# jhbastek/PhysicsInformedDiffusionModels

Measured on NVIDIA H100. Metric: train samples/s Darcy 64x64 PIDM, higher is better.
Workload: dtype bf16

## Files before the change

physicsinformeddiffusionmodels_b200/csrc/attention_fused.cu:

```cuda
#define PIDM_PDL_GROUP 1
#include "common.cuh"
#include "mma_util.cuh"
#include "pidm.h"

namespace pidm {

constexpr int LF_C = 32;

__device__ __forceinline__ uint32_t movm_t(uint32_t x) {
    uint32_t y;
    asm volatile("movmatrix.sync.aligned.m8n8.trans.b16 %0, %1;" : "=r"(y) : "r"(x));
    return y;
}

__device__ __forceinline__ void load_w_frags(uint32_t (&w)[2][4][2], const __nv_bfloat16* __restrict__ Wrows, int lane) {
    const int g = lane >> 2, t = lane & 3;
#pragma unroll
    for (int ks = 0; ks < 2; ++ks)
#pragma unroll
        for (int nt = 0; nt < 4; ++nt) {
            const uint32_t* row = reinterpret_cast<const uint32_t*>(Wrows + (size_t)(nt * 8 + g) * LF_C + ks * 16 + 2 * t);
            w[ks][nt][0] = __ldg(row);
            w[ks][nt][1] = __ldg(row + 4);
        }
}
template <int MT>
__device__ __forceinline__ void load_x_frags(uint32_t (&a)[MT][2][4], const __nv_bfloat16* Xs, int lane) {
#pragma unroll
    for (int mt = 0; mt < MT; ++mt)
#pragma unroll
        for (int ks = 0; ks < 2; ++ks) frag_a_rowmajor(a[mt][ks], Xs, LW_PITCH, mt * 16, ks * 16, lane);
}
template <int MT>
__device__ __forceinline__ void project(float (&c)[MT][4][4], const uint32_t (&a)[MT][2][4], const uint32_t (&w)[2][4][2]) {
#pragma unroll
    for (int mt = 0; mt < MT; ++mt)
#pragma unroll
        for (int nt = 0; nt < 4; ++nt) {
#pragma unroll
            for (int i = 0; i < 4; ++i) c[mt][nt][i] = 0.f;
#pragma unroll
            for (int ks = 0; ks < 2; ++ks) mma_bf16(c[mt][nt], a[mt][ks], w[ks][nt][0], w[ks][nt][1]);
        }
}
__device__ __forceinline__ void frag_softmax(float (&c)[4][4], float mul) {
#pragma unroll
    for (int half = 0; half < 2; ++half) {
        float mx = -INFINITY;
#pragma unroll
        for (int nt = 0; nt < 4; ++nt) mx = fmaxf(mx, fmaxf(c[nt][half * 2], c[nt][half * 2 + 1]));
        mx = fmaxf(mx, __shfl_xor_sync(0xffffffffu, mx, 1));
        mx = fmaxf(mx, __shfl_xor_sync(0xffffffffu, mx, 2));
        float s = 0.f;
#pragma unroll
        for (int nt = 0; nt < 4; ++nt) {
            c[nt][half * 2] = __expf(c[nt][half * 2] - mx);
            c[nt][half * 2 + 1] = __expf(c[nt][half * 2 + 1] - mx);
            s += c[nt][half * 2] + c[nt][half * 2 + 1];
        }
        s += __shfl_xor_sync(0xffffffffu, s, 1);
        s += __shfl_xor_sync(0xffffffffu, s, 2);
        const float inv = mul / s;
#pragma unroll
        for (int nt = 0; nt < 4; ++nt) { c[nt][half * 2] *= inv; c[nt][half * 2 + 1] *= inv; }
    }
}
__device__ __forceinline__ void c_to_a(uint32_t (&a)[2][4], const float (&c)[4][4]) {
#pragma unroll
    for (int ks = 0; ks < 2; ++ks) {
        a[ks][0] = pack_bf16(c[2 * ks][0], c[2 * ks][1]);
        a[ks][1] = pack_bf16(c[2 * ks][2], c[2 * ks][3]);
        a[ks][2] = pack_bf16(c[2 * ks + 1][0], c[2 * ks + 1][1]);
        a[ks][3] = pack_bf16(c[2 * ks + 1][2], c[2 * ks + 1][3]);
    }
}
__device__ __forceinline__ void load_cols(float (&v)[8], const float* __restrict__ src, int lane) {
    const int t = lane & 3;
#pragma unroll
    for (int nt = 0; nt < 4; ++nt) { v[nt * 2] = src[nt * 8 + 2 * t]; v[nt * 2 + 1] = src[nt * 8 + 2 * t + 1]; }
}

constexpr int LFS_STAGES = 2;
__global__ void __launch_bounds__(256) laf_kmax_kernel(const __nv_bfloat16* __restrict__ xn,
                                                       const __nv_bfloat16* __restrict__ W, float* __restrict__ part,
                                                       int N, int rows_per_chunk) {
    pdl_trigger();
    pdl_wait();
    extern __shared__ __align__(16) unsigned char raw[];
    const int b = blockIdx.y, chunk = blockIdx.x, lane = threadIdx.x & 31, h = threadIdx.x >> 5;
    __nv_bfloat16* ring = reinterpret_cast<__nv_bfloat16*>(raw) + (size_t)h * (LFS_STAGES * LW_TILE);
    const int n_begin = chunk * rows_per_chunk, n_end = min(N, n_begin + rows_per_chunk);
    const int n_tiles = (n_end - n_begin) / 32;
    const __nv_bfloat16* xsrc = xn + ((size_t)b * N + n_begin) * LF_C;
    auto issue = [&](int it) {
        if (it < n_tiles) lw_issue<32>(ring + (size_t)(it % LFS_STAGES) * LW_TILE, xsrc + (size_t)it * 32 * LF_C, LF_C, lane);
        cp_commit();
    };
#pragma unroll
    for (int s = 0; s < LFS_STAGES; ++s) issue(s);
    uint32_t wk[2][4][2];
    load_w_frags(wk, W + (size_t)(LM_HID + h * LM_D) * LF_C, lane);
    float m[8];
#pragma unroll
    for (int i = 0; i < 8; ++i) m[i] = -INFINITY;
    for (int it = 0; it < n_tiles; ++it) {
        cp_wait<LFS_STAGES - 1>();
        __syncwarp();
        uint32_t ax[2][2][4];
        load_x_frags<2>(ax, ring + (size_t)(it % LFS_STAGES) * LW_TILE, lane);
        __syncwarp();
        issue(it + LFS_STAGES);
        float ck[2][4][4];
        project<2>(ck, ax, wk);
#pragma unroll
        for (int nt = 0; nt < 4; ++nt)
#pragma unroll
            for (int j = 0; j < 2; ++j)
                m[nt * 2 + j] = fmaxf(fmaxf(m[nt * 2 + j], fmaxf(ck[0][nt][j], ck[0][nt][2 + j])),
                                      fmaxf(ck[1][nt][j], ck[1][nt][2 + j]));
    }
#pragma unroll
    for (int off = 4; off < 32; off <<= 1)
#pragma unroll
        for (int i = 0; i < 8; ++i) m[i] = fmaxf(m[i], __shfl_xor_sync(0xffffffffu, m[i], off));
    if (lane < 4) {
        float* o = part + ((size_t)b * gridDim.x + chunk) * LM_HID + h * LM_D;
#pragma unroll
        for (int nt = 0; nt < 4; ++nt)
#pragma unroll
            for (int j = 0; j < 2; ++j) o[nt * 8 + 2 * lane + j] = m[nt * 2 + j];
    }
}

__global__ void laf_finalize_kernel(float* __restrict__ ctx, float* __restrict__ kzinv, int n_rows) {
    pdl_trigger();
    pdl_wait();
    const int row = blockIdx.x * (blockDim.x / 32) + (threadIdx.x >> 5), lane = threadIdx.x & 31;
    if (row >= n_rows) return;
    const float zi = 1.f / kzinv[row];
    ctx[(size_t)row * LM_D + lane] *= zi;
    __syncwarp();
    if (lane == 0) kzinv[row] = zi;
}

constexpr int LFP_WO_TILE = LF_C * LW_PITCH;

__device__ __forceinline__ void lfp_dout_acc(float (&c)[4][4], const uint32_t (&ady)[2][4], const __nv_bfloat16* Wo, int lane) {
#pragma unroll
    for (int nt = 0; nt < 4; ++nt)
#pragma unroll
        for (int i = 0; i < 4; ++i) c[nt][i] = 0.f;
#pragma unroll
    for (int kc = 0; kc < 2; ++kc)
#pragma unroll
        for (int np = 0; np < 2; ++np) {
            uint32_t bw[4];
            frag_b_krows(bw, Wo, LW_PITCH, kc * 16, np * 16, lane);
            mma_bf16(c[2 * np], ady[kc], bw[0], bw[1]);
            mma_bf16(c[2 * np + 1], ady[kc], bw[2], bw[3]);
        }
}
__device__ __forceinline__ void lfp_dout(uint32_t (&ag)[2][4], const __nv_bfloat16* dyt, const __nv_bfloat16* Wo, int lane) {
    uint32_t ady[2][4];
    frag_a_rowmajor(ady[0], dyt, LW_PITCH, 0, 0, lane);
    frag_a_rowmajor(ady[1], dyt, LW_PITCH, 0, 16, lane);
    float c[4][4];
    lfp_dout_acc(c, ady, Wo, lane);
    c_to_a(ag, c);
}

template <int MODE, bool PROJ = false>
struct LfcCfg {
    static constexpr int STAGES = MODE == 0 ? 4 : 2;
    static constexpr int STAGE_ELEMS = MODE == 0 ? LW_TILE : 2 * LW_TILE;
    static constexpr size_t SMEM = (size_t)LM_HEADS * STAGES * STAGE_ELEMS * 2 + (size_t)LM_HEADS * 2 * LM_D * 4 +
                                   (PROJ ? (size_t)LM_HEADS * LFP_WO_TILE * 2 : 0);
};
template <int MODE, bool PROJ = false>
__global__ void __launch_bounds__(256, 2) laf_ctx_kernel(const __nv_bfloat16* __restrict__ xn, const __nv_bfloat16* __restrict__ W,
                                                      const __nv_bfloat16* __restrict__ dout, const float* __restrict__ part,
                                                      int n_stat_chunks, float* __restrict__ kmax, float* __restrict__ kzinv,
                                                      float* __restrict__ ctx, int N, int chunk_px, float scale,
                                                      const __nv_bfloat16* __restrict__ w_out) {
    static_assert(!PROJ || MODE == 1, "PROJ applies to the dcontext pass");
    pdl_trigger();
    pdl_wait();
    extern __shared__ __align__(16) unsigned char raw[];
    constexpr int LFC_STAGES = LfcCfg<MODE>::STAGES, LFC_STAGE_ELEMS = LfcCfg<MODE>::STAGE_ELEMS;
    const int b = blockIdx.y, chunk = blockIdx.x, lane = threadIdx.x & 31, h = threadIdx.x >> 5;
    __nv_bfloat16* ring = reinterpret_cast<__nv_bfloat16*>(raw) + (size_t)h * (LFC_STAGES * LFC_STAGE_ELEMS);
    float* sM = reinterpret_cast<float*>(raw + (size_t)LM_HEADS * LFC_STAGES * LFC_STAGE_ELEMS * 2) + h * 2 * LM_D;
    float* sZi = sM + LM_D;
    __nv_bfloat16* Wo = reinterpret_cast<__nv_bfloat16*>(raw + LfcCfg<MODE>::SMEM) + h * LFP_WO_TILE;
    const int n_begin = chunk * chunk_px, n_end = min(N, n_begin + chunk_px);
    const int n_tiles = (n_end - n_begin) / 32;
    const size_t pix0 = (size_t)b * N + n_begin;
    const __nv_bfloat16* xsrc = xn + pix0 * LF_C;
    const __nv_bfloat16* gsrc = (MODE == 1) ? (PROJ ? dout + pix0 * LF_C : dout + pix0 * LM_HID + h * LM_D) : nullptr;
    constexpr int G_STRIDE = PROJ ? LF_C : LM_HID;
    if (PROJ) {
        lw_issue<32>(Wo, w_out + h * LM_D, LM_HID, lane);
        cp_commit();
    }
    auto issue = [&](int it) {
        if (it < n_tiles) {
            __nv_bfloat16* buf = ring + (size_t)(it % LFC_STAGES) * LFC_STAGE_ELEMS;
            lw_issue<32>(buf, xsrc + (size_t)it * 32 * LF_C, LF_C, lane);
            if (MODE == 1) lw_issue<32>(buf + LW_TILE, gsrc + (size_t)it * 32 * G_STRIDE, G_STRIDE, lane);
        }
        cp_commit();
    };
#pragma unroll
    for (int s = 0; s < LFC_STAGES; ++s) issue(s);
    uint32_t w0[2][4][2], w1[2][4][2];
    load_w_frags(w0, W + (size_t)((MODE == 0 ? LM_HID : 0) + h * LM_D) * LF_C, lane);
    if (MODE == 0) load_w_frags(w1, W + (size_t)(2 * LM_HID + h * LM_D) * LF_C, lane);
    float Mc[8];
    float zacc[8];
#pragma unroll
    for (int i = 0; i < 8; ++i) zacc[i] = 0.f;
    if (MODE == 0) {
        const int c = h * LM_D + lane;
        float M = -INFINITY;
        for (int i = 0; i < n_stat_chunks; ++i) M = fmaxf(M, part[((size_t)b * n_stat_chunks + i) * LM_HID + c]);
        sM[lane] = M;
        if (chunk == 0) kmax[(size_t)b * LM_HID + c] = M;
        __syncwarp();
        load_cols(Mc, sM, lane);
    }
    float acc[2][4][4];
#pragma unroll
    for (int i = 0; i < 2; ++i)
#pragma unroll
        for (int j = 0; j < 4; ++j)
#pragma unroll
            for (int k = 0; k < 4; ++k) acc[i][j][k] = 0.f;
    for (int it = 0; it < n_tiles; ++it) {
        cp_wait<LFC_STAGES - 1>();
        __syncwarp();
        const __nv_bfloat16* buf = ring + (size_t)(it % LFC_STAGES) * LFC_STAGE_ELEMS;
        uint32_t ax[2][2][4];
        load_x_frags<2>(ax, buf, lane);
        uint32_t bv[2][4][2];
        if (PROJ) {
#pragma unroll
            for (int mt = 0; mt < 2; ++mt) {
                uint32_t ady[2][4];
                frag_a_rowmajor(ady[0], buf + LW_TILE, LW_PITCH, mt * 16, 0, lane);
                frag_a_rowmajor(ady[1], buf + LW_TILE, LW_PITCH, mt * 16, 16, lane);
                float cd[4][4];
                lfp_dout_acc(cd, ady, Wo, lane);
#pragma unroll
                for (int nt = 0; nt < 4; ++nt) {
                    bv[mt][nt][0] = movm_t(pack_bf16(cd[nt][0], cd[nt][1]));
                    bv[mt][nt][1] = movm_t(pack_bf16(cd[nt][2], cd[nt][3]));
                }
            }
        } else if (MODE == 1) {
#pragma unroll
            for (int ks = 0; ks < 2; ++ks) {
                uint32_t b01[4], b23[4];
                frag_b_krows(b01, buf + LW_TILE, LW_PITCH, ks * 16, 0, lane);
                frag_b_krows(b23, buf + LW_TILE, LW_PITCH, ks * 16, 16, lane);
                bv[ks][0][0] = b01[0]; bv[ks][0][1] = b01[1]; bv[ks][1][0] = b01[2]; bv[ks][1][1] = b01[3];
                bv[ks][2][0] = b23[0]; bv[ks][2][1] = b23[1]; bv[ks][3][0] = b23[2]; bv[ks][3][1] = b23[3];
            }
        }
        __syncwarp();
        issue(it + LFC_STAGES);
        float cw[2][4][4];
        project<2>(cw, ax, w0);
        if (MODE == 0) {
#pragma unroll
            for (int mt = 0; mt < 2; ++mt)
#pragma unroll
                for (int nt = 0; nt < 4; ++nt)
#pragma unroll
                    for (int i = 0; i < 4; ++i) {
                        cw[mt][nt][i] = __expf(cw[mt][nt][i] - Mc[nt * 2 + (i & 1)]);
                        zacc[nt * 2 + (i & 1)] += cw[mt][nt][i];
                    }
            float cv[2][4][4];
            project<2>(cv, ax, w1);
#pragma unroll
            for (int mt = 0; mt < 2; ++mt)
#pragma unroll
                for (int nt = 0; nt < 4; ++nt) {
                    bv[mt][nt][0] = movm_t(pack_bf16(cv[mt][nt][0], cv[mt][nt][1]));
                    bv[mt][nt][1] = movm_t(pack_bf16(cv[mt][nt][2], cv[mt][nt][3]));
                }
        } else {
            frag_softmax(cw[0], scale);
            frag_softmax(cw[1], scale);
        }
#pragma unroll
        for (int mt = 0; mt < 2; ++mt) {
#pragma unroll
            for (int md = 0; md < 2; ++md) {
                uint32_t a[4];
                a[0] = movm_t(pack_bf16(cw[mt][2 * md][0], cw[mt][2 * md][1]));
                a[1] = movm_t(pack_bf16(cw[mt][2 * md + 1][0], cw[mt][2 * md + 1][1]));
                a[2] = movm_t(pack_bf16(cw[mt][2 * md][2], cw[mt][2 * md][3]));
                a[3] = movm_t(pack_bf16(cw[mt][2 * md + 1][2], cw[mt][2 * md + 1][3]));
#pragma unroll
                for (int ne = 0; ne < 4; ++ne) mma_bf16(acc[md][ne], a, bv[mt][ne][0], bv[mt][ne][1]);
            }
        }
    }
    const int g = lane >> 2, t = lane & 3;
    if (MODE == 0) {
#pragma unroll
        for (int off = 4; off < 32; off <<= 1)
#pragma unroll
            for (int i = 0; i < 8; ++i) zacc[i] += __shfl_xor_sync(0xffffffffu, zacc[i], off);
        if (lane < 4) {
#pragma unroll
            for (int nt = 0; nt < 4; ++nt)
#pragma unroll
                for (int j = 0; j < 2; ++j)
                    atomicAdd(kzinv + (size_t)b * LM_HID + h * LM_D + nt * 8 + 2 * lane + j, zacc[nt * 2 + j]);
        }
    }
    float* cb = ctx + ((size_t)b * LM_HEADS + h) * LM_D * LM_D;
#pragma unroll
    for (int md = 0; md < 2; ++md)
#pragma unroll
        for (int half = 0; half < 2; ++half) {
            const int d = md * 16 + g + half * 8;
            const float f = (MODE == 0) ? 1.f / (float)N : 1.f;
#pragma unroll
            for (int ne = 0; ne < 4; ++ne) {
                const int e = ne * 8 + 2 * t;
                atomicAdd(cb + d * LM_D + e, acc[md][ne][half * 2] * f);
                atomicAdd(cb + d * LM_D + e + 1, acc[md][ne][half * 2 + 1] * f);
            }
        }
}

constexpr int LFO_STAGES = 2;
constexpr int LFOP_STAGES = 3;
constexpr int LFO_R_PITCH = LF_C + 8;
constexpr size_t LAF_OUT_PROJ_SMEM = (size_t)LFOP_STAGES * LW_TILE * 2 + (size_t)LM_HEADS * LFP_WO_TILE * 2 +
                                     (size_t)LM_HEADS * 32 * LFO_R_PITCH * 4;
template <bool PROJ = false>
__global__ void __launch_bounds__(256) laf_out_kernel(const __nv_bfloat16* __restrict__ xn, const __nv_bfloat16* __restrict__ W,
                                                      const float* __restrict__ ctx, __nv_bfloat16* __restrict__ out, int N,
                                                      int chunk_px, float scale, const __nv_bfloat16* __restrict__ w_out,
                                                      const float* __restrict__ b_out,
                                                      const __nv_bfloat16* __restrict__ residual) {
    pdl_trigger();
    pdl_wait();
    extern __shared__ __align__(16) unsigned char raw[];
    constexpr int STAGES = PROJ ? LFOP_STAGES : LFO_STAGES;
    const int b = blockIdx.y, chunk = blockIdx.x, lane = threadIdx.x & 31, h = threadIdx.x >> 5;
    __nv_bfloat16* ring = reinterpret_cast<__nv_bfloat16*>(raw) + (PROJ ? 0 : (size_t)h * ((LFO_STAGES + 1) * LW_TILE));
    __nv_bfloat16* Os = ring + LFO_STAGES * LW_TILE;
    __nv_bfloat16* Wo = reinterpret_cast<__nv_bfloat16*>(raw) + LFOP_STAGES * LW_TILE + h * LFP_WO_TILE;
    float* R = reinterpret_cast<float*>(reinterpret_cast<__nv_bfloat16*>(raw) + LFOP_STAGES * LW_TILE +
                                        LM_HEADS * LFP_WO_TILE);
    const int n_begin = chunk * chunk_px, n_end = min(N, n_begin + chunk_px);
    const int n_tiles = (n_end - n_begin) / 32;
    const size_t pix0 = (size_t)b * N + n_begin;
    const __nv_bfloat16* xsrc = xn + pix0 * LF_C;
    __nv_bfloat16* odst = out + pix0 * LM_HID + h * LM_D;
    if (PROJ) {
        lw_issue<32>(Wo, w_out + h * LM_D, LM_HID, lane);
        cp_commit();
    }
    auto issue = [&](int it) {
        if (it < n_tiles && (!PROJ || h == 0))
            lw_issue<32>(ring + (size_t)(it % STAGES) * LW_TILE, xsrc + (size_t)it * 32 * LF_C, LF_C, lane);
        cp_commit();
    };
#pragma unroll
    for (int s = 0; s < (PROJ ? STAGES - 1 : STAGES); ++s) issue(s);
    uint32_t wq[2][4][2];
    load_w_frags(wq, W + (size_t)(h * LM_D) * LF_C, lane);
    const float* ch = ctx + ((size_t)b * LM_HEADS + h) * LM_D * LM_D;
    uint32_t bf[2][4][2];
#pragma unroll
    for (int ks = 0; ks < 2; ++ks)
#pragma unroll
        for (int nt = 0; nt < 4; ++nt) frag_b_global<true>(bf[ks][nt], ch, ks * 16, nt * 8, lane);
    const int g = lane >> 2, t = lane & 3;
    const int rrow = threadIdx.x >> 4, rcol = (threadIdx.x & 15) * 2;
    float2 bias = make_float2(0.f, 0.f);
    if (PROJ) bias = make_float2(b_out[rcol], b_out[rcol + 1]);
    float* Rw = R + h * 32 * LFO_R_PITCH;
    for (int it = 0; it < n_tiles; ++it) {
        uint32_t ax[2][2][4];
        if (PROJ) {
            cp_wait<STAGES - 2>();
            __syncthreads();
            issue(it + STAGES - 1);
            load_x_frags<2>(ax, ring + (size_t)(it % STAGES) * LW_TILE, lane);
        } else {
            cp_wait<LFO_STAGES - 1>();
            __syncwarp();
            load_x_frags<2>(ax, ring + (size_t)(it % LFO_STAGES) * LW_TILE, lane);
            __syncwarp();
            issue(it + LFO_STAGES);
        }
        __nv_bfloat162 res[2];
        if (PROJ)
#pragma unroll
            for (int rh = 0; rh < 2; ++rh)
                res[rh] = *reinterpret_cast<const __nv_bfloat162*>(residual + (pix0 + (size_t)it * 32 + rrow + rh * 16) * LF_C + rcol);
        float cq[2][4][4];
        project<2>(cq, ax, wq);
#pragma unroll
        for (int mt = 0; mt < 2; ++mt) {
            frag_softmax(cq[mt], scale);
            uint32_t a[2][4];
            c_to_a(a, cq[mt]);
            float c[4][4];
#pragma unroll
            for (int i = 0; i < 4; ++i)
#pragma unroll
                for (int k = 0; k < 4; ++k) c[i][k] = 0.f;
#pragma unroll
            for (int ks = 0; ks < 2; ++ks)
#pragma unroll
                for (int nt = 0; nt < 4; ++nt) mma_bf16(c[nt], a[ks], bf[ks][nt][0], bf[ks][nt][1]);
            if (PROJ) {
                c_to_a(a, c);
                float y[4][4];
#pragma unroll
                for (int i = 0; i < 4; ++i)
#pragma unroll
                    for (int k = 0; k < 4; ++k) y[i][k] = 0.f;
#pragma unroll
                for (int ke = 0; ke < 2; ++ke)
#pragma unroll
                    for (int np = 0; np < 2; ++np) {
                        uint32_t bw[4];
                        frag_b_nrows(bw, Wo, LW_PITCH, np * 16, ke * 16, lane);
                        mma_bf16(y[2 * np], a[ke], bw[0], bw[1]);
                        mma_bf16(y[2 * np + 1], a[ke], bw[2], bw[3]);
                    }
#pragma unroll
                for (int nt = 0; nt < 4; ++nt)
#pragma unroll
                    for (int half = 0; half < 2; ++half)
                        *reinterpret_cast<float2*>(Rw + (mt * 16 + g + half * 8) * LFO_R_PITCH + nt * 8 + 2 * t) =
                            make_float2(y[nt][half * 2], y[nt][half * 2 + 1]);
            } else {
#pragma unroll
                for (int nt = 0; nt < 4; ++nt) {
                    __nv_bfloat16* o = Os + (size_t)(mt * 16 + g) * LW_PITCH + nt * 8 + 2 * t;
                    *reinterpret_cast<uint32_t*>(o) = pack_bf16(c[nt][0], c[nt][1]);
                    *reinterpret_cast<uint32_t*>(o + 8 * LW_PITCH) = pack_bf16(c[nt][2], c[nt][3]);
                }
            }
        }
        if (PROJ) {
            __syncthreads();
#pragma unroll
            for (int rh = 0; rh < 2; ++rh) {
                const int row = rrow + rh * 16;
                const size_t pix = pix0 + (size_t)it * 32 + row;
                const float2 x = __bfloat1622float2(res[rh]);
                float sx = x.x + bias.x, sy = x.y + bias.y;
#pragma unroll
                for (int w = 0; w < LM_HEADS; ++w) {
                    const float2 v = *reinterpret_cast<const float2*>(R + (w * 32 + row) * LFO_R_PITCH + rcol);
                    sx += v.x;
                    sy += v.y;
                }
                *reinterpret_cast<uint32_t*>(out + pix * LF_C + rcol) = pack_bf16(sx, sy);
            }
        } else {
            __syncwarp();
            lw_store<32>(odst + (size_t)it * 32 * LM_HID, LM_HID, Os, lane);
            __syncwarp();
        }
    }
}

constexpr int LFB_ROWS = 16;
constexpr int LFB_STAGES = 4;
constexpr int LFB_TILE = LFB_ROWS * LW_PITCH;

struct LfbTile {
    uint32_t ax[1][2][4], ag[2][4];
};
__device__ __forceinline__ void lfb_dq(float (&dq)[4][4], const LfbTile& tl, const uint32_t (&wq)[2][4][2],
                                       const uint32_t (&bc)[2][4][2], float scale) {
    float c1[1][4][4], c2[4][4];
    project<1>(c1, tl.ax, wq);
    frag_softmax(c1[0], 1.f);
#pragma unroll
    for (int nt = 0; nt < 4; ++nt) {
#pragma unroll
        for (int i = 0; i < 4; ++i) c2[nt][i] = 0.f;
#pragma unroll
        for (int ks = 0; ks < 2; ++ks) mma_bf16(c2[nt], tl.ag[ks], bc[ks][nt][0], bc[ks][nt][1]);
    }
#pragma unroll
    for (int half = 0; half < 2; ++half) {
        float dot = 0.f;
#pragma unroll
        for (int nt = 0; nt < 4; ++nt)
            dot += c1[0][nt][half * 2] * c2[nt][half * 2] + c1[0][nt][half * 2 + 1] * c2[nt][half * 2 + 1];
        dot += __shfl_xor_sync(0xffffffffu, dot, 1);
        dot += __shfl_xor_sync(0xffffffffu, dot, 2);
#pragma unroll
        for (int nt = 0; nt < 4; ++nt)
#pragma unroll
            for (int j = 0; j < 2; ++j) dq[nt][half * 2 + j] = scale * c1[0][nt][half * 2 + j] * (c2[nt][half * 2 + j] - dot);
    }
}
__device__ __forceinline__ void lfb_dkdv(float (&dk)[4][4], float (&dv)[4][4], const uint32_t (&ax)[1][2][4],
                                         const uint32_t (&wk)[2][4][2], const uint32_t (&wv)[2][4][2],
                                         const uint32_t (&bd)[2][4][2], const uint32_t (&bt)[2][4][2],
                                         const float (&Mc)[8], const float (&Zc)[8], const float (&cdc)[8], float invN) {
    float c1[1][4][4];
    uint32_t a[2][4];
    project<1>(c1, ax, wv);
    c_to_a(a, c1[0]);
#pragma unroll
    for (int nt = 0; nt < 4; ++nt) {
#pragma unroll
        for (int i = 0; i < 4; ++i) dk[nt][i] = 0.f;
#pragma unroll
        for (int ks = 0; ks < 2; ++ks) mma_bf16(dk[nt], a[ks], bd[ks][nt][0], bd[ks][nt][1]);
    }
    project<1>(c1, ax, wk);
#pragma unroll
    for (int nt = 0; nt < 4; ++nt)
#pragma unroll
        for (int i = 0; i < 4; ++i) {
            c1[0][nt][i] = __expf(c1[0][nt][i] - Mc[nt * 2 + (i & 1)]) * Zc[nt * 2 + (i & 1)];
            dk[nt][i] = c1[0][nt][i] * (dk[nt][i] * invN - cdc[nt * 2 + (i & 1)]);
        }
    c_to_a(a, c1[0]);
#pragma unroll
    for (int nt = 0; nt < 4; ++nt) {
#pragma unroll
        for (int i = 0; i < 4; ++i) dv[nt][i] = 0.f;
#pragma unroll
        for (int ks = 0; ks < 2; ++ks) mma_bf16(dv[nt], a[ks], bt[ks][nt][0], bt[ks][nt][1]);
#pragma unroll
        for (int i = 0; i < 4; ++i) dv[nt][i] *= invN;
    }
}
__device__ __forceinline__ void lfb_cd(float (&cdc)[8], float* scd, const float* __restrict__ cg, const float* __restrict__ dg,
                                       int lane) {
    float s = 0.f;
#pragma unroll
    for (int e = 0; e < LM_D; e += 4) {
        const float4 x = *reinterpret_cast<const float4*>(dg + lane * LM_D + e);
        const float4 y = *reinterpret_cast<const float4*>(cg + lane * LM_D + e);
        s += x.x * y.x + x.y * y.y + x.z * y.z + x.w * y.w;
    }
    scd[lane] = s;
    __syncwarp();
    load_cols(cdc, scd, lane);
}

constexpr int LFB_W_PITCH = LF_C + 8;
constexpr int LFB_R_PITCH = LF_C + 8;
template <bool PROJ>
struct LfbCfg {
    static constexpr int STAGE_ELEMS = (PROJ ? 2 : 1 + LM_HEADS) * LFB_TILE;
    static constexpr size_t SMEM_BASE = (size_t)LFB_STAGES * STAGE_ELEMS * 2 + (size_t)3 * LM_HID * LFB_W_PITCH * 2 +
                                        (size_t)LM_HEADS * LFB_ROWS * LFB_R_PITCH * 4 + (size_t)LM_HEADS * LM_D * 4;
    static constexpr size_t SMEM = SMEM_BASE + (PROJ ? (size_t)LM_HEADS * LFP_WO_TILE * 2 : 0);
};

__device__ __forceinline__ void mma_w(float (&c)[4][4], const uint32_t (&g)[2][4], const __nv_bfloat16* Wh, int lane) {
#pragma unroll
    for (int kd = 0; kd < 2; ++kd)
#pragma unroll
        for (int np = 0; np < 2; ++np) {
            uint32_t bw[4];
            frag_b_krows(bw, Wh, LFB_W_PITCH, kd * 16, np * 16, lane);
            mma_bf16(c[2 * np], g[kd], bw[0], bw[1]);
            mma_bf16(c[2 * np + 1], g[kd], bw[2], bw[3]);
        }
}

template <bool PROJ = false>
__global__ void __launch_bounds__(256) laf_bwd_kernel(const __nv_bfloat16* __restrict__ xn, const __nv_bfloat16* __restrict__ W,
                                                      const __nv_bfloat16* __restrict__ dout, const float* __restrict__ ctx,
                                                      const float* __restrict__ dctx, const float* __restrict__ kmax,
                                                      const float* __restrict__ kzinv, __nv_bfloat16* __restrict__ dxn,
                                                      int N, int chunk_px, float scale, const __nv_bfloat16* __restrict__ w_out) {
    pdl_trigger();
    pdl_wait();
    extern __shared__ __align__(16) unsigned char raw[];
    constexpr int LFB_STAGE_ELEMS = LfbCfg<PROJ>::STAGE_ELEMS;
    const int b = blockIdx.y, chunk = blockIdx.x, lane = threadIdx.x & 31, h = threadIdx.x >> 5;
    __nv_bfloat16* ring = reinterpret_cast<__nv_bfloat16*>(raw);
    __nv_bfloat16* Ws = ring + LFB_STAGES * LFB_STAGE_ELEMS;
    __nv_bfloat16* Wo = reinterpret_cast<__nv_bfloat16*>(raw + LfbCfg<PROJ>::SMEM_BASE) + h * LFP_WO_TILE;
    float* R = reinterpret_cast<float*>(Ws + 3 * LM_HID * LFB_W_PITCH);
    float* scd = R + LM_HEADS * LFB_ROWS * LFB_R_PITCH + h * LM_D;
    const int n_begin = chunk * chunk_px, n_end = min(N, n_begin + chunk_px);
// ... 116 lines not shown
        for (int np = 0; np < 2; ++np) {
            mma_bf16(acc[md][2 * np], a, bx[np][0], bx[np][1]);
            mma_bf16(acc[md][2 * np + 1], a, bx[np][2], bx[np][3]);
        }
    }
}

template <int PART, bool PROJ = false>
__global__ void __launch_bounds__(256) laf_wgrad_kernel(const __nv_bfloat16* __restrict__ xn, const __nv_bfloat16* __restrict__ W,
                                                        const __nv_bfloat16* __restrict__ dout, const float* __restrict__ ctx,
                                                        const float* __restrict__ dctx, const float* __restrict__ kmax,
                                                        const float* __restrict__ kzinv, float* __restrict__ grad_w, int N,
                                                        int chunk_px, long long w_stride_n, long long w_stride_c, float scale,
                                                        const __nv_bfloat16* __restrict__ w_out, float* __restrict__ grad_wo,
                                                        long long wo_stride_n, long long wo_stride_c) {
    pdl_trigger();
    pdl_wait();
    extern __shared__ __align__(16) unsigned char raw[];
    using Cfg = LfwCfg<PART, PROJ>;
    constexpr int MATS = Cfg::MATS, STAGE_ELEMS = Cfg::STAGE_ELEMS, S_PITCH = Cfg::S_PITCH;
    const int b = blockIdx.y, chunk = blockIdx.x, lane = threadIdx.x & 31, h = threadIdx.x >> 5;
    __nv_bfloat16* ring = reinterpret_cast<__nv_bfloat16*>(raw) + (size_t)h * (LFB_STAGES * STAGE_ELEMS);
    float* scd = reinterpret_cast<float*>(raw + (size_t)LM_HEADS * LFB_STAGES * STAGE_ELEMS * 2) + h * LM_D;
    __nv_bfloat16* Wo = reinterpret_cast<__nv_bfloat16*>(raw + Cfg::SMEM_BASE) + h * LFP_WO_TILE;
    const int n_begin = chunk * chunk_px, n_end = min(N, n_begin + chunk_px);
    const int n_tiles = (n_end - n_begin) / LFB_ROWS;
    const size_t pix0 = (size_t)b * N + n_begin;
    const __nv_bfloat16* xsrc = xn + pix0 * LF_C;
    const __nv_bfloat16* gsrc = PROJ ? dout + pix0 * LF_C : dout + pix0 * LM_HID + h * LM_D;
    constexpr int G_STRIDE = PROJ ? LF_C : LM_HID;
    if (PROJ) {
        lw_issue<32>(Wo, w_out + h * LM_D, LM_HID, lane);
        cp_commit();
    }
    auto issue = [&](int it) {
        if (it < n_tiles) {
            __nv_bfloat16* buf = ring + (size_t)(it % LFB_STAGES) * STAGE_ELEMS;
            lw_issue<LFB_ROWS>(buf, xsrc + (size_t)it * LFB_ROWS * LF_C, LF_C, lane);
            if (PART == 0) lw_issue<LFB_ROWS>(buf + LFB_TILE, gsrc + (size_t)it * LFB_ROWS * G_STRIDE, G_STRIDE, lane);
        }
        cp_commit();
    };
#pragma unroll
    for (int s = 0; s < LFB_STAGES; ++s) issue(s);
    const float* cg = ctx + ((size_t)b * LM_HEADS + h) * LM_D * LM_D;
    const float* dg = dctx + ((size_t)b * LM_HEADS + h) * LM_D * LM_D;
    float Mc[8], Zc[8], cdc[8];
    uint32_t w0[2][4][2], w1[2][4][2];
    uint32_t b0[2][4][2], b1[2][4][2];
    if (PART == 0) {
        load_w_frags(w0, W + (size_t)(h * LM_D) * LF_C, lane);
    } else {
        lfb_cd(cdc, scd, cg, dg, lane);
        load_cols(Mc, kmax + (size_t)b * LM_HID + h * LM_D, lane);
        load_cols(Zc, kzinv + (size_t)b * LM_HID + h * LM_D, lane);
        load_w_frags(w0, W + (size_t)(LM_HID + h * LM_D) * LF_C, lane);
        load_w_frags(w1, W + (size_t)(2 * LM_HID + h * LM_D) * LF_C, lane);
    }
#pragma unroll
    for (int ks = 0; ks < 2; ++ks)
#pragma unroll
        for (int nt = 0; nt < 4; ++nt) {
            frag_b_global<false>(b0[ks][nt], PART == 0 ? cg : dg, ks * 16, nt * 8, lane);
            if (PART == 1 || PROJ) frag_b_global<true>(b1[ks][nt], PART == 1 ? dg : cg, ks * 16, nt * 8, lane);
        }
    const float invN = 1.f / (float)N;
    float acc[MATS][2][4][4];
#pragma unroll
    for (int m = 0; m < MATS; ++m)
#pragma unroll
        for (int i = 0; i < 2; ++i)
#pragma unroll
            for (int j = 0; j < 4; ++j)
#pragma unroll
                for (int k = 0; k < 4; ++k) acc[m][i][j][k] = 0.f;
    for (int it = 0; it < n_tiles; ++it) {
        cp_wait<LFB_STAGES - 1>();
        __syncwarp();
        const __nv_bfloat16* buf = ring + (size_t)(it % LFB_STAGES) * STAGE_ELEMS;
        LfbTile tl;
        load_x_frags<1>(tl.ax, buf, lane);
        uint32_t bx[2][4];
        frag_b_krows(bx[0], buf, LW_PITCH, 0, 0, lane);
        frag_b_krows(bx[1], buf, LW_PITCH, 0, 16, lane);
        uint32_t ady[2][4], bdy[2][4];
        if (PROJ) {
            frag_a_rowmajor(ady[0], buf + LFB_TILE, LW_PITCH, 0, 0, lane);
            frag_a_rowmajor(ady[1], buf + LFB_TILE, LW_PITCH, 0, 16, lane);
            frag_b_krows(bdy[0], buf + LFB_TILE, LW_PITCH, 0, 0, lane);
            frag_b_krows(bdy[1], buf + LFB_TILE, LW_PITCH, 0, 16, lane);
        } else if (PART == 0) {
            frag_a_rowmajor(tl.ag[0], buf + LFB_TILE, LW_PITCH, 0, 0, lane);
            frag_a_rowmajor(tl.ag[1], buf + LFB_TILE, LW_PITCH, 0, 16, lane);
        }
        __syncwarp();
        issue(it + LFB_STAGES);
        if (PART == 0) {
            if (PROJ) {
                float c[4][4];
                lfp_dout_acc(c, ady, Wo, lane);
                c_to_a(tl.ag, c);
            }
            float dq[4][4];
            lfb_dq(dq, tl, w0, b0, scale);
            acc_gtx(acc[0], dq, bx);
            if (PROJ) {
                float cq[1][4][4], o[4][4];
                project<1>(cq, tl.ax, w0);
                frag_softmax(cq[0], scale);
                uint32_t a[2][4];
                c_to_a(a, cq[0]);
#pragma unroll
                for (int nt = 0; nt < 4; ++nt) {
#pragma unroll
                    for (int i = 0; i < 4; ++i) o[nt][i] = 0.f;
#pragma unroll
                    for (int ks = 0; ks < 2; ++ks) mma_bf16(o[nt], a[ks], b1[ks][nt][0], b1[ks][nt][1]);
                }
                acc_gtx(acc[MATS - 1], o, bdy);
            }
        } else {
            float dk[4][4], dv[4][4];
            lfb_dkdv(dk, dv, tl.ax, w0, w1, b0, b1, Mc, Zc, cdc, invN);
            acc_gtx(acc[0], dk, bx);
            acc_gtx(acc[MATS - 1], dv, bx);
        }
    }
    cp_wait<0>();
    __syncwarp();
    float* S = reinterpret_cast<float*>(ring);
    const int g = lane >> 2, t = lane & 3;
#pragma unroll
    for (int m = 0; m < MATS; ++m) {
#pragma unroll
        for (int md = 0; md < 2; ++md)
#pragma unroll
            for (int nc = 0; nc < 4; ++nc)
#pragma unroll
                for (int i = 0; i < 4; ++i) S[(md * 16 + g + 8 * (i >> 1)) * S_PITCH + nc * 8 + 2 * t + (i & 1)] = acc[m][md][nc][i];
        __syncwarp();
        if (PROJ && m == 1) {
            float* dst = grad_wo + (long long)(h * LM_D + lane) * wo_stride_c;
#pragma unroll 4
            for (int c = 0; c < LF_C; ++c) atomicAdd(dst + c * wo_stride_n, S[lane * S_PITCH + c]);
        } else {
            float* dst = grad_w + (long long)((PART + m) * LM_HID + h * LM_D) * w_stride_n + lane * w_stride_c;
#pragma unroll 4
            for (int d = 0; d < LM_D; ++d) atomicAdd(dst + d * w_stride_n, S[d * S_PITCH + lane]);
        }
        __syncwarp();
    }
}

constexpr size_t LAF_STATS_SMEM = (size_t)LM_HEADS * LFS_STAGES * LW_TILE * 2;
constexpr size_t LAF_OUT_SMEM = (size_t)LM_HEADS * (LFO_STAGES + 1) * LW_TILE * 2;

static int laf_attrs() {
    static bool done = false;
    if (!done) {
        PIDM_CUDA(cudaFuncSetAttribute(laf_kmax_kernel, cudaFuncAttributeMaxDynamicSharedMemorySize, (int)LAF_STATS_SMEM));
        PIDM_CUDA(cudaFuncSetAttribute(laf_ctx_kernel<0>, cudaFuncAttributeMaxDynamicSharedMemorySize, (int)LfcCfg<0>::SMEM));
        PIDM_CUDA(cudaFuncSetAttribute(laf_ctx_kernel<1>, cudaFuncAttributeMaxDynamicSharedMemorySize, (int)LfcCfg<1>::SMEM));
        PIDM_CUDA(cudaFuncSetAttribute(laf_ctx_kernel<1, true>, cudaFuncAttributeMaxDynamicSharedMemorySize, (int)LfcCfg<1, true>::SMEM));
        PIDM_CUDA(cudaFuncSetAttribute(laf_out_kernel<false>, cudaFuncAttributeMaxDynamicSharedMemorySize, (int)LAF_OUT_SMEM));
        PIDM_CUDA(cudaFuncSetAttribute(laf_out_kernel<true>, cudaFuncAttributeMaxDynamicSharedMemorySize, (int)LAF_OUT_PROJ_SMEM));
        PIDM_CUDA(cudaFuncSetAttribute(laf_bwd_kernel<false>, cudaFuncAttributeMaxDynamicSharedMemorySize, (int)LfbCfg<false>::SMEM));
        PIDM_CUDA(cudaFuncSetAttribute(laf_bwd_kernel<true>, cudaFuncAttributeMaxDynamicSharedMemorySize, (int)LfbCfg<true>::SMEM));
        PIDM_CUDA(cudaFuncSetAttribute(laf_wgrad_kernel<0>, cudaFuncAttributeMaxDynamicSharedMemorySize, (int)LfwCfg<0>::SMEM));
        PIDM_CUDA(cudaFuncSetAttribute(laf_wgrad_kernel<0, true>, cudaFuncAttributeMaxDynamicSharedMemorySize, (int)LfwCfg<0, true>::SMEM));
        PIDM_CUDA(cudaFuncSetAttribute(laf_wgrad_kernel<1>, cudaFuncAttributeMaxDynamicSharedMemorySize, (int)LfwCfg<1>::SMEM));
        done = true;
    }
    return 0;
}

static int laf_chunk_px(int B, int N, int ctas_per_sm) {
    int k = (num_sms() * ctas_per_sm) / B;
    if (k < 1) k = 1;
    int px = ((N + k - 1) / k + 31) / 32 * 32;
    if (px < 64) px = 64;
    if (px > N) px = N;
    return px;
}
static int laf_stat_chunks(int N) {
    int c = N / 128;
    if (c < 1) c = 1;
    if (c > 16) c = 16;
    return c;
}

template <bool PROJ>
static int laf_fwd(const void* xn, const void* w_qkv, const void* w_out, const float* b_out, const void* residual, void* out,
                   float* ctx, float* kmax, float* kzinv, float* workspace, int B, int N, void* stream) {
    PIDM_REQUIRE(N % 128 == 0, "linattn_fused: N must be a multiple of 128 (got %d)", N);
    cudaStream_t st = (cudaStream_t)stream;
    if (int e = laf_attrs()) return e;
    const float scale = 0.17677669529663687f;
    const __nv_bfloat16* x = (const __nv_bfloat16*)xn;
    const __nv_bfloat16* w = (const __nv_bfloat16*)w_qkv;
    PIDM_CUDA(cudaMemsetAsync(ctx, 0, (size_t)B * LM_HEADS * LM_D * LM_D * sizeof(float), st));
    PIDM_CUDA(cudaMemsetAsync(kzinv, 0, (size_t)B * LM_HID * sizeof(float), st));
    const int chunks = laf_stat_chunks(N);
    const int rpc = N / chunks;
    PIDM_REQUIRE(rpc % 32 == 0 && rpc * chunks == N, "linattn_fused: bad statistics chunking for N=%d", N);
    PIDM_CUDA(launch_pdl(laf_kmax_kernel, dim3(dim3(chunks, B)), dim3(256), (size_t)(LAF_STATS_SMEM), st, x, w, workspace, N, rpc));
    const int cpx = laf_chunk_px(B, N, 2);
    PIDM_CUDA(launch_pdl(laf_ctx_kernel<0>, dim3(dim3((N + cpx - 1) / cpx, B)), dim3(256), (size_t)(LfcCfg<0>::SMEM), st, x, w, nullptr, workspace, chunks, kmax, kzinv,
                                                                             ctx, N, cpx, scale, nullptr));
    PIDM_CUDA(launch_pdl(laf_finalize_kernel, dim3((B * LM_HID + 7) / 8), dim3(256), (size_t)(0), st, ctx, kzinv, B * LM_HID));
    const int opx = laf_chunk_px(B, N, PROJ ? 2 : 3);
    PIDM_CUDA(launch_pdl(laf_out_kernel<PROJ>, dim3(dim3((N + opx - 1) / opx, B)), dim3(256),
                         PROJ ? LAF_OUT_PROJ_SMEM : LAF_OUT_SMEM, st, x, w, ctx, (__nv_bfloat16*)out, N, opx, scale,
                         (const __nv_bfloat16*)w_out, b_out, (const __nv_bfloat16*)residual));
    PIDM_LAUNCH_CHECK("linattn_fused_fwd");
    return 0;
}

template <bool PROJ>
static int laf_bwd(const void* xn, const void* w_qkv, const void* w_out, const void* dout, const float* ctx,
                   const float* kmax, const float* kzinv, void* dxn, float* dctx, int B, int N, void* stream) {
    PIDM_REQUIRE(N % 128 == 0, "linattn_fused: N must be a multiple of 128 (got %d)", N);
    cudaStream_t st = (cudaStream_t)stream;
    if (int e = laf_attrs()) return e;
    const float scale = 0.17677669529663687f;
    const __nv_bfloat16* x = (const __nv_bfloat16*)xn;
    const __nv_bfloat16* w = (const __nv_bfloat16*)w_qkv;
    const __nv_bfloat16* wo = (const __nv_bfloat16*)w_out;
    PIDM_CUDA(cudaMemsetAsync(dctx, 0, (size_t)B * LM_HEADS * LM_D * LM_D * sizeof(float), st));
    const int cpx = laf_chunk_px(B, N, 2);
    PIDM_CUDA(launch_pdl(laf_ctx_kernel<1, PROJ>, dim3(dim3((N + cpx - 1) / cpx, B)), dim3(256), LfcCfg<1, PROJ>::SMEM, st, x, w,
                         (const __nv_bfloat16*)dout, nullptr, 0, nullptr, nullptr, dctx, N, cpx, scale, wo));
    const int bpx = laf_chunk_px(B, N, 1);
    PIDM_CUDA(launch_pdl(laf_bwd_kernel<PROJ>, dim3(dim3((N + bpx - 1) / bpx, B)), dim3(256), LfbCfg<PROJ>::SMEM, st, x, w,
                         (const __nv_bfloat16*)dout, ctx, dctx, kmax, kzinv, (__nv_bfloat16*)dxn, N, bpx, scale, wo));
    PIDM_LAUNCH_CHECK("linattn_fused_bwd");
    return 0;
}

template <bool PROJ>
static int laf_wgrad(const void* xn, const void* w_qkv, const void* w_out, const void* dout, const float* ctx,
                     const float* dctx, const float* kmax, const float* kzinv, float* grad_w, long long w_stride_n,
                     long long w_stride_c, float* grad_wo, long long wo_stride_n, long long wo_stride_c, int B, int N,
                     void* stream) {
    PIDM_REQUIRE(N % 128 == 0, "linattn_fused: N must be a multiple of 128 (got %d)", N);
    cudaStream_t st = (cudaStream_t)stream;
    if (int e = laf_attrs()) return e;
    const float scale = 0.17677669529663687f;
    const __nv_bfloat16* x = (const __nv_bfloat16*)xn;
    const __nv_bfloat16* w = (const __nv_bfloat16*)w_qkv;
    const __nv_bfloat16* wo = (const __nv_bfloat16*)w_out;
    const __nv_bfloat16* g = (const __nv_bfloat16*)dout;
    const int px = laf_chunk_px(B, N, 1);
    const dim3 grid((N + px - 1) / px, B);
    PIDM_CUDA(launch_pdl(laf_wgrad_kernel<0, PROJ>, grid, dim3(256), LfwCfg<0, PROJ>::SMEM, st, x, w, g, ctx, dctx, kmax, kzinv,
                         grad_w, N, px, w_stride_n, w_stride_c, scale, wo, grad_wo, wo_stride_n, wo_stride_c));
    PIDM_CUDA(launch_pdl(laf_wgrad_kernel<1>, grid, dim3(256), LfwCfg<1>::SMEM, st, x, w, g, ctx, dctx, kmax, kzinv, grad_w, N,
                         px, w_stride_n, w_stride_c, scale, nullptr, nullptr, 0LL, 0LL));
    PIDM_LAUNCH_CHECK("linattn_fused_wgrad");
    return 0;
}

}
using namespace pidm;

extern "C" int pidm_linattn_fused_supported(int C, int heads, int N, int dtype) {
    return (C == LF_C && heads == LM_HEADS && dtype == PIDM_BF16 && N % 128 == 0) ? 1 : 0;
}

extern "C" int pidm_linattn_fused_workspace_floats(int B, int N) { return B * laf_stat_chunks(N) * LM_HID; }

extern "C" int pidm_linattn_fused_plan(int B, int N, int* out) {
    PIDM_REQUIRE(N % 128 == 0 && B > 0, "linattn_fused_plan: N must be a multiple of 128 (got %d)", N);
    const int v[5] = {laf_stat_chunks(N), laf_chunk_px(B, N, 2), laf_chunk_px(B, N, 3), laf_chunk_px(B, N, 1),
                      laf_chunk_px(B, N, 1)};
    for (int i = 0; i < 5; ++i) out[i] = v[i];
    return 0;
}

extern "C" int pidm_linattn_fused_fwd(const void* xn, const void* w_qkv, void* out, float* ctx, float* kmax, float* kzinv,
                                      float* workspace, int B, int N, void* stream) {
    return laf_fwd<false>(xn, w_qkv, nullptr, nullptr, nullptr, out, ctx, kmax, kzinv, workspace, B, N, stream);
}

extern "C" int pidm_linattn_fused_bwd(const void* xn, const void* w_qkv, const void* dout, const float* ctx,
                                      const float* kmax, const float* kzinv, void* dxn, float* dctx, int B, int N,
                                      void* stream) {
    return laf_bwd<false>(xn, w_qkv, nullptr, dout, ctx, kmax, kzinv, dxn, dctx, B, N, stream);
}

extern "C" int pidm_linattn_fused_wgrad(const void* xn, const void* w_qkv, const void* dout, const float* ctx,
                                        const float* dctx, const float* kmax, const float* kzinv, float* grad_w, int B,
                                        int N, long long w_stride_n, long long w_stride_c, void* stream) {
    return laf_wgrad<false>(xn, w_qkv, nullptr, dout, ctx, dctx, kmax, kzinv, grad_w, w_stride_n, w_stride_c, nullptr, 0, 0,
                            B, N, stream);
}

extern "C" int pidm_linattn_block_fwd(const void* xn, const void* w_qkv, const void* w_out, const float* b_out,
                                      const void* residual, void* y, float* ctx, float* kmax, float* kzinv,
                                      float* workspace, int B, int N, void* stream) {
    PIDM_REQUIRE(w_out && b_out && residual, "linattn_block_fwd: w_out, b_out and residual are required");
    return laf_fwd<true>(xn, w_qkv, w_out, b_out, residual, y, ctx, kmax, kzinv, workspace, B, N, stream);
}

extern "C" int pidm_linattn_block_bwd(const void* xn, const void* w_qkv, const void* w_out, const void* dy, const float* ctx,
                                      const float* kmax, const float* kzinv, void* dxn, float* dctx, int B, int N,
                                      void* stream) {
    return laf_bwd<true>(xn, w_qkv, w_out, dy, ctx, kmax, kzinv, dxn, dctx, B, N, stream);
}

extern "C" int pidm_linattn_block_wgrad(const void* xn, const void* w_qkv, const void* w_out, const void* dy,
                                        const float* ctx, const float* dctx, const float* kmax, const float* kzinv,
                                        float* grad_w_qkv, long long qkv_stride_n, long long qkv_stride_c,
                                        float* grad_w_out, long long out_stride_n, long long out_stride_c, int B, int N,
                                        void* stream) {
    return laf_wgrad<true>(xn, w_qkv, w_out, dy, ctx, dctx, kmax, kzinv, grad_w_qkv, qkv_stride_n, qkv_stride_c,
                           grad_w_out, out_stride_n, out_stride_c, B, N, stream);
}
```

Before: 7018.

## Fold output projection into context, share kmax ring across warps, interleave ctx passes

After: 7080, median of 6. About the same (+0.9%).

```diff
diff --git a/physicsinformeddiffusionmodels_b200/csrc/attention_fused.cu b/physicsinformeddiffusionmodels_b200/csrc/attention_fused.cu
--- a/physicsinformeddiffusionmodels_b200/csrc/attention_fused.cu
+++ b/physicsinformeddiffusionmodels_b200/csrc/attention_fused.cu
@@ -80,7 +80,7 @@
     for (int nt = 0; nt < 4; ++nt) { v[nt * 2] = src[nt * 8 + 2 * t]; v[nt * 2 + 1] = src[nt * 8 + 2 * t + 1]; }
 }
 
-constexpr int LFS_STAGES = 2;
+constexpr int LFS_STAGES = 6;
 __global__ void __launch_bounds__(256) laf_kmax_kernel(const __nv_bfloat16* __restrict__ xn,
                                                        const __nv_bfloat16* __restrict__ W, float* __restrict__ part,
                                                        int N, int rows_per_chunk) {
@@ -88,28 +88,28 @@
     pdl_wait();
     extern __shared__ __align__(16) unsigned char raw[];
     const int b = blockIdx.y, chunk = blockIdx.x, lane = threadIdx.x & 31, h = threadIdx.x >> 5;
-    __nv_bfloat16* ring = reinterpret_cast<__nv_bfloat16*>(raw) + (size_t)h * (LFS_STAGES * LW_TILE);
+    __nv_bfloat16* ring = reinterpret_cast<__nv_bfloat16*>(raw);
     const int n_begin = chunk * rows_per_chunk, n_end = min(N, n_begin + rows_per_chunk);
     const int n_tiles = (n_end - n_begin) / 32;
     const __nv_bfloat16* xsrc = xn + ((size_t)b * N + n_begin) * LF_C;
     auto issue = [&](int it) {
-        if (it < n_tiles) lw_issue<32>(ring + (size_t)(it % LFS_STAGES) * LW_TILE, xsrc + (size_t)it * 32 * LF_C, LF_C, lane);
+        if (it < n_tiles && h == 0)
+            lw_issue<32>(ring + (size_t)(it % LFS_STAGES) * LW_TILE, xsrc + (size_t)it * 32 * LF_C, LF_C, lane);
         cp_commit();
     };
 #pragma unroll
-    for (int s = 0; s < LFS_STAGES; ++s) issue(s);
+    for (int s = 0; s < LFS_STAGES - 1; ++s) issue(s);
     uint32_t wk[2][4][2];
     load_w_frags(wk, W + (size_t)(LM_HID + h * LM_D) * LF_C, lane);
     float m[8];
 #pragma unroll
     for (int i = 0; i < 8; ++i) m[i] = -INFINITY;
     for (int it = 0; it < n_tiles; ++it) {
-        cp_wait<LFS_STAGES - 1>();
-        __syncwarp();
+        cp_wait<LFS_STAGES - 2>();
+        __syncthreads();
+        issue(it + LFS_STAGES - 1);
         uint32_t ax[2][2][4];
         load_x_frags<2>(ax, ring + (size_t)(it % LFS_STAGES) * LW_TILE, lane);
-        __syncwarp();
-        issue(it + LFS_STAGES);
         float ck[2][4][4];
         project<2>(ck, ax, wk);
 #pragma unroll
@@ -169,6 +169,41 @@
     c_to_a(ag, c);
 }
 
+__device__ __forceinline__ void lfp_g_frags(uint32_t (&bg)[2][4][2], const float* __restrict__ ch,
+                                            const __nv_bfloat16* __restrict__ w_out, int h, int lane) {
+    const int g = lane >> 2, t = lane & 3;
+    uint32_t wo[2][4][2];
+#pragma unroll
+    for (int ks = 0; ks < 2; ++ks)
+#pragma unroll
+        for (int nt = 0; nt < 4; ++nt) {
+            const uint32_t* row =
+                reinterpret_cast<const uint32_t*>(w_out + (size_t)(nt * 8 + g) * LM_HID + h * LM_D + ks * 16 + 2 * t);
+            wo[ks][nt][0] = __ldg(row);
+            wo[ks][nt][1] = __ldg(row + 4);
+        }
+#pragma unroll
+    for (int mt = 0; mt < 2; ++mt) {
+        uint32_t a[2][4];
+#pragma unroll
+        for (int ks = 0; ks < 2; ++ks)
+#pragma unroll
+            for (int i = 0; i < 4; ++i) {
+                const float2 v = *reinterpret_cast<const float2*>(ch + (mt * 16 + g + 8 * (i & 1)) * LM_D + ks * 16 + 2 * t +
+                                                                  8 * (i >> 1));
+                a[ks][i] = pack_bf16(v.x, v.y);
+            }
+#pragma unroll
+        for (int nt = 0; nt < 4; ++nt) {
+            float c[4] = {0.f, 0.f, 0.f, 0.f};
+#pragma unroll
+            for (int ks = 0; ks < 2; ++ks) mma_bf16(c, a[ks], wo[ks][nt][0], wo[ks][nt][1]);
+            bg[mt][nt][0] = movm_t(pack_bf16(c[0], c[1]));
+            bg[mt][nt][1] = movm_t(pack_bf16(c[2], c[3]));
+        }
+    }
+}
+
 template <int MODE, bool PROJ = false>
 struct LfcCfg {
     static constexpr int STAGES = MODE == 0 ? 4 : 2;
@@ -176,6 +211,18 @@
     static constexpr size_t SMEM = (size_t)LM_HEADS * STAGES * STAGE_ELEMS * 2 + (size_t)LM_HEADS * 2 * LM_D * 4 +
                                    (PROJ ? (size_t)LM_HEADS * LFP_WO_TILE * 2 : 0);
 };
+__device__ __forceinline__ void acc_wtv(float (&acc)[2][4][4], const float (&w)[4][4], const uint32_t (&bv)[4][2]) {
+#pragma unroll
+    for (int md = 0; md < 2; ++md) {
+        uint32_t a[4];
+        a[0] = movm_t(pack_bf16(w[2 * md][0], w[2 * md][1]));
+        a[1] = movm_t(pack_bf16(w[2 * md + 1][0], w[2 * md + 1][1]));
+        a[2] = movm_t(pack_bf16(w[2 * md][2], w[2 * md][3]));
+        a[3] = movm_t(pack_bf16(w[2 * md + 1][2], w[2 * md + 1][3]));
+#pragma unroll
+        for (int ne = 0; ne < 4; ++ne) mma_bf16(acc[md][ne], a, bv[ne][0], bv[ne][1]);
+    }
+}
 template <int MODE, bool PROJ = false>
 __global__ void __launch_bounds__(256, 2) laf_ctx_kernel(const __nv_bfloat16* __restrict__ xn, const __nv_bfloat16* __restrict__ W,
                                                       const __nv_bfloat16* __restrict__ dout, const float* __restrict__ part,
@@ -268,43 +315,34 @@
         }
         __syncwarp();
         issue(it + LFC_STAGES);
-        float cw[2][4][4];
-        project<2>(cw, ax, w0);
         if (MODE == 0) {
 #pragma unroll
-            for (int mt = 0; mt < 2; ++mt)
+            for (int mt = 0; mt < 2; ++mt) {
+                const uint32_t(&am)[1][2][4] = *reinterpret_cast<const uint32_t(*)[1][2][4]>(&ax[mt]);
+                float ck[1][4][4], cv[1][4][4];
+                project<1>(ck, am, w0);
 #pragma unroll
                 for (int nt = 0; nt < 4; ++nt)
 #pragma unroll
                     for (int i = 0; i < 4; ++i) {
-                        cw[mt][nt][i] = __expf(cw[mt][nt][i] - Mc[nt * 2 + (i & 1)]);
-                        zacc[nt * 2 + (i & 1)] += cw[mt][nt][i];
+                        ck[0][nt][i] = __expf(ck[0][nt][i] - Mc[nt * 2 + (i & 1)]);
+                        zacc[nt * 2 + (i & 1)] += ck[0][nt][i];
                     }
-            float cv[2][4][4];
-            project<2>(cv, ax, w1);
-#pragma unroll
-            for (int mt = 0; mt < 2; ++mt)
+                project<1>(cv, am, w1);
 #pragma unroll
                 for (int nt = 0; nt < 4; ++nt) {
-                    bv[mt][nt][0] = movm_t(pack_bf16(cv[mt][nt][0], cv[mt][nt][1]));
-                    bv[mt][nt][1] = movm_t(pack_bf16(cv[mt][nt][2], cv[mt][nt][3]));
+                    bv[mt][nt][0] = movm_t(pack_bf16(cv[0][nt][0], cv[0][nt][1]));
+                    bv[mt][nt][1] = movm_t(pack_bf16(cv[0][nt][2], cv[0][nt][3]));
                 }
+                acc_wtv(acc, ck[0], bv[mt]);
+            }
         } else {
+            float cw[2][4][4];
+            project<2>(cw, ax, w0);
             frag_softmax(cw[0], scale);
             frag_softmax(cw[1], scale);
-        }
-#pragma unroll
-        for (int mt = 0; mt < 2; ++mt) {
-#pragma unroll
-            for (int md = 0; md < 2; ++md) {
-                uint32_t a[4];
-                a[0] = movm_t(pack_bf16(cw[mt][2 * md][0], cw[mt][2 * md][1]));
-                a[1] = movm_t(pack_bf16(cw[mt][2 * md + 1][0], cw[mt][2 * md + 1][1]));
-                a[2] = movm_t(pack_bf16(cw[mt][2 * md][2], cw[mt][2 * md][3]));
-                a[3] = movm_t(pack_bf16(cw[mt][2 * md + 1][2], cw[mt][2 * md + 1][3]));
-#pragma unroll
-                for (int ne = 0; ne < 4; ++ne) mma_bf16(acc[md][ne], a, bv[mt][ne][0], bv[mt][ne][1]);
-            }
+#pragma unroll
+            for (int mt = 0; mt < 2; ++mt) acc_wtv(acc, cw[mt], bv[mt]);
         }
     }
     const int g = lane >> 2, t = lane & 3;
@@ -340,8 +378,7 @@
 constexpr int LFO_STAGES = 2;
 constexpr int LFOP_STAGES = 3;
 constexpr int LFO_R_PITCH = LF_C + 8;
-constexpr size_t LAF_OUT_PROJ_SMEM = (size_t)LFOP_STAGES * LW_TILE * 2 + (size_t)LM_HEADS * LFP_WO_TILE * 2 +
-                                     (size_t)LM_HEADS * 32 * LFO_R_PITCH * 4;
+constexpr size_t LAF_OUT_PROJ_SMEM = (size_t)LFOP_STAGES * LW_TILE * 2 + (size_t)LM_HEADS * 32 * LFO_R_PITCH * 4;
 template <bool PROJ = false>
 __global__ void __launch_bounds__(256) laf_out_kernel(const __nv_bfloat16* __restrict__ xn, const __nv_bfloat16* __restrict__ W,
                                                       const float* __restrict__ ctx, __nv_bfloat16* __restrict__ out, int N,
@@ -355,18 +392,12 @@
     const int b = blockIdx.y, chunk = blockIdx.x, lane = threadIdx.x & 31, h = threadIdx.x >> 5;
     __nv_bfloat16* ring = reinterpret_cast<__nv_bfloat16*>(raw) + (PROJ ? 0 : (size_t)h * ((LFO_STAGES + 1) * LW_TILE));
     __nv_bfloat16* Os = ring + LFO_STAGES * LW_TILE;
-    __nv_bfloat16* Wo = reinterpret_cast<__nv_bfloat16*>(raw) + LFOP_STAGES * LW_TILE + h * LFP_WO_TILE;
-    float* R = reinterpret_cast<float*>(reinterpret_cast<__nv_bfloat16*>(raw) + LFOP_STAGES * LW_TILE +
-                                        LM_HEADS * LFP_WO_TILE);
+    float* R = reinterpret_cast<float*>(reinterpret_cast<__nv_bfloat16*>(raw) + LFOP_STAGES * LW_TILE);
     const int n_begin = chunk * chunk_px, n_end = min(N, n_begin + chunk_px);
     const int n_tiles = (n_end - n_begin) / 32;
     const size_t pix0 = (size_t)b * N + n_begin;
     const __nv_bfloat16* xsrc = xn + pix0 * LF_C;
     __nv_bfloat16* odst = out + pix0 * LM_HID + h * LM_D;
-    if (PROJ) {
-        lw_issue<32>(Wo, w_out + h * LM_D, LM_HID, lane);
-        cp_commit();
-    }
     auto issue = [&](int it) {
         if (it < n_tiles && (!PROJ || h == 0))
             lw_issue<32>(ring + (size_t)(it % STAGES) * LW_TILE, xsrc + (size_t)it * 32 * LF_C, LF_C, lane);
@@ -378,10 +409,14 @@
     load_w_frags(wq, W + (size_t)(h * LM_D) * LF_C, lane);
     const float* ch = ctx + ((size_t)b * LM_HEADS + h) * LM_D * LM_D;
     uint32_t bf[2][4][2];
-#pragma unroll
-    for (int ks = 0; ks < 2; ++ks)
-#pragma unroll
-        for (int nt = 0; nt < 4; ++nt) frag_b_global<true>(bf[ks][nt], ch, ks * 16, nt * 8, lane);
+    if (PROJ) {
+        lfp_g_frags(bf, ch, w_out, h, lane);
+    } else {
+#pragma unroll
+        for (int ks = 0; ks < 2; ++ks)
+#pragma unroll
+            for (int nt = 0; nt < 4; ++nt) frag_b_global<true>(bf[ks][nt], ch, ks * 16, nt * 8, lane);
+    }
     const int g = lane >> 2, t = lane & 3;
     const int rrow = threadIdx.x >> 4, rcol = (threadIdx.x & 15) * 2;
     float2 bias = make_float2(0.f, 0.f);
@@ -423,27 +458,12 @@
 #pragma unroll
                 for (int nt = 0; nt < 4; ++nt) mma_bf16(c[nt], a[ks], bf[ks][nt][0], bf[ks][nt][1]);
             if (PROJ) {
-                c_to_a(a, c);
-                float y[4][4];
-#pragma unroll
-                for (int i = 0; i < 4; ++i)
-#pragma unroll
-                    for (int k = 0; k < 4; ++k) y[i][k] = 0.f;
-#pragma unroll
-                for (int ke = 0; ke < 2; ++ke)
-#pragma unroll
-                    for (int np = 0; np < 2; ++np) {
-                        uint32_t bw[4];
-                        frag_b_nrows(bw, Wo, LW_PITCH, np * 16, ke * 16, lane);
-                        mma_bf16(y[2 * np], a[ke], bw[0], bw[1]);
-                        mma_bf16(y[2 * np + 1], a[ke], bw[2], bw[3]);
-                    }
 #pragma unroll
                 for (int nt = 0; nt < 4; ++nt)
 #pragma unroll
                     for (int half = 0; half < 2; ++half)
                         *reinterpret_cast<float2*>(Rw + (mt * 16 + g + half * 8) * LFO_R_PITCH + nt * 8 + 2 * t) =
-                            make_float2(y[nt][half * 2], y[nt][half * 2 + 1]);
+                            make_float2(c[nt][half * 2], c[nt][half * 2 + 1]);
             } else {
 #pragma unroll
                 for (int nt = 0; nt < 4; ++nt) {
@@ -866,7 +886,7 @@
     }
 }
 
-constexpr size_t LAF_STATS_SMEM = (size_t)LM_HEADS * LFS_STAGES * LW_TILE * 2;
+constexpr size_t LAF_STATS_SMEM = (size_t)LFS_STAGES * LW_TILE * 2;
 constexpr size_t LAF_OUT_SMEM = (size_t)LM_HEADS * (LFO_STAGES + 1) * LW_TILE * 2;
 
 static int laf_attrs() {
@@ -922,7 +942,7 @@
     PIDM_CUDA(launch_pdl(laf_ctx_kernel<0>, dim3(dim3((N + cpx - 1) / cpx, B)), dim3(256), (size_t)(LfcCfg<0>::SMEM), st, x, w, nullptr, workspace, chunks, kmax, kzinv,
                                                                              ctx, N, cpx, scale, nullptr));
     PIDM_CUDA(launch_pdl(laf_finalize_kernel, dim3((B * LM_HID + 7) / 8), dim3(256), (size_t)(0), st, ctx, kzinv, B * LM_HID));
-    const int opx = laf_chunk_px(B, N, PROJ ? 2 : 3);
+    const int opx = laf_chunk_px(B, N, 3);
     PIDM_CUDA(launch_pdl(laf_out_kernel<PROJ>, dim3(dim3((N + opx - 1) / opx, B)), dim3(256),
                          PROJ ? LAF_OUT_PROJ_SMEM : LAF_OUT_SMEM, st, x, w, ctx, (__nv_bfloat16*)out, N, opx, scale,
                          (const __nv_bfloat16*)w_out, b_out, (const __nv_bfloat16*)residual));
```
